# nekStab/neklab

Measured on AMD Instinct MI355X. Metric: linop matvecs/sec + Arnoldi iter time, E=10k N=7, 1/2/4/8 GPU, higher is better.
Workload: dtype f64

## Files before the change

### include/neklab_gpu.h

```cpp
#ifndef NEKLAB_GPU_H
#define NEKLAB_GPU_H

#include <stddef.h>
#include <stdint.h>

#ifdef __cplusplus
extern "C" {
#endif

typedef struct nlg_ctx nlg_ctx;
typedef struct nlg_mesh nlg_mesh;
typedef struct nlg_vec nlg_vec;
typedef struct nlg_basis nlg_basis;
typedef struct nlg_linop nlg_linop;

enum { NLG_VX = 0, NLG_VY = 1, NLG_VZ = 2, NLG_PR = 3, NLG_THETA = 4  };

const char *nlg_last_error(void);
int nlg_version(void);
int nlg_ctx_create(int device, nlg_ctx **out);
int nlg_ctx_destroy(nlg_ctx *ctx);
int nlg_ctx_sync(nlg_ctx *ctx);
int nlg_comm_unique_id(void *out128);
int nlg_ctx_comm_init(nlg_ctx *ctx, int rank, int nranks, const void *unique_id128);
int nlg_ctx_rank(const nlg_ctx *ctx, int *rank, int *nranks);
int nlg_ctx_comm_init_shm(nlg_ctx *ctx, int rank, int nranks, const char *name, int64_t slot_bytes);
int64_t nlg_halo_plan(int rank, int nranks, const int64_t *counts, const int64_t *labels_concat,
                      int64_t *neigh_counts, int64_t *shared_out, int64_t capacity);
int64_t nlg_halo_boundary_labels(int n, int dim, int64_t E, const int64_t *glo, int64_t *labels_out, int64_t capacity);
int64_t nlg_halo_lists(int n, int dim, int64_t E, const int64_t *glo, int rank, int nranks, const int64_t *counts,
                       const int64_t *labels_concat, int64_t *neigh_counts, int32_t *send_idx, int64_t cap_send,
                       int32_t *roff, int32_t *rpos, int32_t *coff, int32_t *cidx, int64_t cap_copies, int64_t *nlab_out);
int nlg_prof_enable(nlg_ctx *ctx, int class_mask);
int nlg_prof_sample(nlg_ctx *ctx, int stride);
int nlg_prof_reset(nlg_ctx *ctx);
int nlg_prof_get(nlg_ctx *ctx, const char *name, int64_t *count, double *total_ms);
int nlg_counters(int64_t *launches, int64_t *collectives);

typedef struct nlg_mesh_desc {
    int dim;
    int n;
    int lxd;
    int64_t nelv;
    const double *xm1;
    const double *ym1;
    const double *zm1;
    const int64_t *glo_num;
    const int64_t *lglel;
    const double *v1mask;
    const double *v2mask;
    const double *v3mask;
    const double *tmask;
    int has_outflow;
} nlg_mesh_desc;

int nlg_mesh_create(nlg_ctx *ctx, const nlg_mesh_desc *desc, nlg_mesh **out);
int nlg_mesh_destroy(nlg_mesh *mesh);
int nlg_mesh_sizes(const nlg_mesh *mesh, int64_t *lvn, int64_t *lpn, int *dim, int *n);
int nlg_mesh_get(const nlg_mesh *mesh, const char *name, double *out, int64_t count);

int nlg_vec_create(nlg_mesh *mesh, int nscal, int lorder, nlg_vec **out);
int nlg_vec_destroy(nlg_vec *v);
int nlg_vec_generation(const nlg_vec *v, int64_t *gen);
int nlg_vec_release(nlg_vec *v);
int nlg_vec_adopt(nlg_vec *v, int64_t gen, int *status);
int nlg_vec_pin(nlg_vec *v, int64_t gen);
int nlg_vec_unpin(nlg_vec *v, int64_t gen);
int nlg_vec_pool_limit(int64_t bytes);
int nlg_vec_pool_trim(int64_t *freed_bytes);
int nlg_vec_clone(const nlg_vec *src, nlg_vec **out);
int nlg_vec_copy(nlg_vec *dst, const nlg_vec *src);
int nlg_vec_zero(nlg_vec *self);
int nlg_vec_rand(nlg_vec *self, int ifnorm, uint64_t seed);
int nlg_vec_rand_noise(nlg_vec *self, uint64_t seed);
int nlg_vec_rand_finish(nlg_vec *self, int ifnorm);
int nlg_vec_scal(nlg_vec *self, double alpha);
int nlg_vec_axpby(double alpha, const nlg_vec *vec, double beta, nlg_vec *self);
int nlg_vec_dot(const nlg_vec *self, const nlg_vec *vec, double *out);
int nlg_vec_norm(const nlg_vec *self, double *out);
int nlg_vec_size(const nlg_vec *self, int64_t *out);
int64_t nlg_vec_size_value(const nlg_vec *self);
int nlg_vec_has_rst_value(const nlg_vec *self);
int64_t nlg_vec_size_checked(const nlg_vec *self, int64_t gen);
int nlg_vec_has_rst_checked(const nlg_vec *self, int64_t gen);
int nlg_vec_outpost(const nlg_vec *self, const char *path, int with_coords, double time, int istep);
int nlg_vec_save_rst(nlg_vec *self, const nlg_vec *vec_rst, int irst);
int nlg_vec_get_rst(const nlg_vec *self, nlg_vec *vec_rst, int irst);
int nlg_vec_has_rst_fields(const nlg_vec *self, int *out);
int nlg_vec_clear_rst_fields(nlg_vec *self);
int nlg_vec_nrst(const nlg_vec *self, int *out);
int nlg_vec_set_field(nlg_vec *self, int field, int irst, const double *host, int64_t count);
int nlg_vec_get_field(const nlg_vec *self, int field, int irst, double *host, int64_t count);
int nlg_set_axpby_rst_consistent(int flag);

int nlg_basis_create(nlg_mesh *mesh, int nscal, int lorder, int nvec, nlg_basis **out);
int nlg_basis_destroy(nlg_basis *b);
int nlg_basis_vec(nlg_basis *b, int i, nlg_vec **out);
int nlg_basis_block_dot(const nlg_basis *b, int k, const nlg_vec *w, double *h);
int nlg_basis_block_axpy(const nlg_basis *b, int k, const double *h, nlg_vec *w);
int nlg_basis_cgs2(const nlg_basis *b, int k, nlg_vec *w, double *h, double *beta);
int nlg_basis_block_cgs2(nlg_basis *b, int k, int s, double *coef);
int nlg_basis_last_block_rank(const nlg_basis *b, int *rank);
int nlg_basis_combine(const nlg_basis *b, int k, const double *c, nlg_vec *out);

typedef struct nlg_exptA_config {
    double tau;
    double re;
    double cfl_limit;
    double vtol;
    double ptol;
    double dt;
    int torder;
// ... 96 lines not shown
```

### neklab_amd/_lib.py

```python
from __future__ import annotations

import ctypes as C
import os

HERE = os.path.dirname(os.path.abspath(__file__))
LIB_PATH = os.path.join(HERE, "libneklab_gpu.so")

c_double_p = C.POINTER(C.c_double)
c_int64_p = C.POINTER(C.c_int64)
c_int_p = C.POINTER(C.c_int)
vp = C.c_void_p


class NlgError(RuntimeError):
    pass


class MeshDesc(C.Structure):
    _fields_ = [
        ("dim", C.c_int), ("n", C.c_int), ("lxd", C.c_int), ("nelv", C.c_int64),
        ("xm1", c_double_p), ("ym1", c_double_p), ("zm1", c_double_p),
        ("glo_num", c_int64_p), ("lglel", c_int64_p),
        ("v1mask", c_double_p), ("v2mask", c_double_p), ("v3mask", c_double_p), ("tmask", c_double_p),
        ("has_outflow", C.c_int),
# ... 7 lines not shown
        ("torder", C.c_int), ("maxit_v", C.c_int), ("maxit_p", C.c_int),
        ("fixed_iters_v", C.c_int), ("fixed_iters_p", C.c_int), ("pprecond", C.c_int), ("pproj", C.c_int),
        ("ifheat", C.c_int), ("conductivity", C.c_double), ("rhocp", C.c_double), ("buoy", C.c_double * 3),
        ("no_history", C.c_int),
        ("filter_weight", C.c_double), ("filter_modes", C.c_int),
    ]


class EigsOpts(C.Structure):
    _fields_ = [
        ("kdim", C.c_int), ("transpose", C.c_int), ("max_restarts", C.c_int), ("write_intermediate", C.c_int),
        ("tol", C.c_double), ("logfile", C.c_char_p), ("seed", C.c_uint64), ("block_size", C.c_int), ("warm_start", C.c_int),
    ]


class OtdOpts(C.Structure):
    _fields_ = [("r", C.c_int), ("startstep", C.c_int), ("orthostep", C.c_int), ("trans", C.c_int), ("solve_baseflow", C.c_int)]


SIGNATURES = {
    "nlg_last_error": (C.c_char_p, []),
    "nlg_version": (C.c_int, []),
    "nlg_ctx_create": (C.c_int, [C.c_int, C.POINTER(vp)]),
    "nlg_ctx_destroy": (C.c_int, [vp]),
    "nlg_ctx_sync": (C.c_int, [vp]),
    "nlg_comm_unique_id": (C.c_int, [vp]),
    "nlg_ctx_comm_init": (C.c_int, [vp, C.c_int, C.c_int, vp]),
    "nlg_ctx_rank": (C.c_int, [vp, c_int_p, c_int_p]),
    "nlg_ctx_comm_init_shm": (C.c_int, [vp, C.c_int, C.c_int, C.c_char_p, C.c_int64]),
    "nlg_halo_plan": (C.c_int64, [C.c_int, C.c_int, c_int64_p, c_int64_p, c_int64_p, c_int64_p, C.c_int64]),
    "nlg_halo_boundary_labels": (C.c_int64, [C.c_int, C.c_int, C.c_int64, c_int64_p, c_int64_p, C.c_int64]),
    "nlg_halo_lists": (C.c_int64, [C.c_int, C.c_int, C.c_int64, c_int64_p, C.c_int, C.c_int, c_int64_p, c_int64_p, c_int64_p,
                                   C.POINTER(C.c_int32), C.c_int64, C.POINTER(C.c_int32), C.POINTER(C.c_int32), C.POINTER(C.c_int32),
                                   C.POINTER(C.c_int32), C.c_int64, c_int64_p]),
    "nlg_prof_enable": (C.c_int, [vp, C.c_int]),
    "nlg_prof_sample": (C.c_int, [vp, C.c_int]),
    "nlg_prof_reset": (C.c_int, [vp]),
    "nlg_prof_get": (C.c_int, [vp, C.c_char_p, c_int64_p, c_double_p]),
    "nlg_counters": (C.c_int, [c_int64_p, c_int64_p]),
    "nlg_basis_last_block_rank": (C.c_int, [vp, C.POINTER(C.c_int)]),
    "nlg_vec_generation": (C.c_int, [vp, c_int64_p]),
    "nlg_vec_release": (C.c_int, [vp]),
    "nlg_vec_adopt": (C.c_int, [vp, C.c_int64, C.POINTER(C.c_int)]),
    "nlg_vec_pin": (C.c_int, [vp, C.c_int64]),
    "nlg_vec_unpin": (C.c_int, [vp, C.c_int64]),
    "nlg_vec_size_checked": (C.c_int64, [vp, C.c_int64]),
    "nlg_vec_has_rst_checked": (C.c_int, [vp, C.c_int64]),
    "nlg_vec_pool_limit": (C.c_int, [C.c_int64]),
    "nlg_vec_pool_trim": (C.c_int, [c_int64_p]),
    "nlg_mesh_create": (C.c_int, [vp, C.POINTER(MeshDesc), C.POINTER(vp)]),
    "nlg_mesh_destroy": (C.c_int, [vp]),
    "nlg_mesh_sizes": (C.c_int, [vp, c_int64_p, c_int64_p, c_int_p, c_int_p]),
    "nlg_mesh_get": (C.c_int, [vp, C.c_char_p, c_double_p, C.c_int64]),
    "nlg_vec_create": (C.c_int, [vp, C.c_int, C.c_int, C.POINTER(vp)]),
    "nlg_vec_destroy": (C.c_int, [vp]),
    "nlg_vec_clone": (C.c_int, [vp, C.POINTER(vp)]),
    "nlg_vec_copy": (C.c_int, [vp, vp]),
    "nlg_vec_zero": (C.c_int, [vp]),
    "nlg_vec_rand": (C.c_int, [vp, C.c_int, C.c_uint64]),
    "nlg_vec_rand_noise": (C.c_int, [vp, C.c_uint64]),
    "nlg_vec_size_value": (C.c_int64, [vp]),
    "nlg_vec_has_rst_value": (C.c_int, [vp]),
    "nlg_basis_block_cgs2": (C.c_int, [vp, C.c_int, C.c_int, c_double_p]),
    "nlg_linop_matvec_block": (C.c_int, [vp, C.c_int, C.POINTER(vp), C.POINTER(vp), C.c_int]),
    "nlg_block_arnoldi_step": (C.c_int, [vp, vp, C.c_int, C.c_int, c_double_p, C.c_int, C.c_int]),
    "nlg_vec_outpost": (C.c_int, [vp, C.c_char_p, C.c_int, C.c_double, C.c_int]),
    "nlg_vec_rand_finish": (C.c_int, [vp, C.c_int]),
    "nlg_vec_scal": (C.c_int, [vp, C.c_double]),
    "nlg_vec_axpby": (C.c_int, [C.c_double, vp, C.c_double, vp]),
    "nlg_vec_dot": (C.c_int, [vp, vp, c_double_p]),
    "nlg_vec_norm": (C.c_int, [vp, c_double_p]),
    "nlg_vec_size": (C.c_int, [vp, c_int64_p]),
    "nlg_vec_save_rst": (C.c_int, [vp, vp, C.c_int]),
    "nlg_vec_get_rst": (C.c_int, [vp, vp, C.c_int]),
    "nlg_vec_has_rst_fields": (C.c_int, [vp, c_int_p]),
    "nlg_vec_clear_rst_fields": (C.c_int, [vp]),
    "nlg_vec_nrst": (C.c_int, [vp, c_int_p]),
    "nlg_vec_set_field": (C.c_int, [vp, C.c_int, C.c_int, c_double_p, C.c_int64]),
    "nlg_vec_get_field": (C.c_int, [vp, C.c_int, C.c_int, c_double_p, C.c_int64]),
    "nlg_set_axpby_rst_consistent": (C.c_int, [C.c_int]),
    "nlg_basis_create": (C.c_int, [vp, C.c_int, C.c_int, C.c_int, C.POINTER(vp)]),
    "nlg_basis_destroy": (C.c_int, [vp]),
    "nlg_basis_vec": (C.c_int, [vp, C.c_int, C.POINTER(vp)]),
    "nlg_basis_block_dot": (C.c_int, [vp, C.c_int, vp, c_double_p]),
    "nlg_basis_block_axpy": (C.c_int, [vp, C.c_int, c_double_p, vp]),
    "nlg_basis_cgs2": (C.c_int, [vp, C.c_int, vp, c_double_p, c_double_p]),
    "nlg_basis_combine": (C.c_int, [vp, C.c_int, c_double_p, vp]),
    "nlg_exptA_config_default": (C.c_int, [C.POINTER(ExptAConfig)]),
    "nlg_linop_create": (C.c_int, [vp, C.POINTER(ExptAConfig), vp, C.POINTER(vp)]),
    "nlg_linop_destroy": (C.c_int, [vp]),
    "nlg_linop_init": (C.c_int, [vp]),
    "nlg_linop_nonlinear_map": (C.c_int, [vp, vp, vp]),
    "nlg_linop_set_baseflow": (C.c_int, [vp, vp]),
    "nlg_linop_set_tolerances": (C.c_int, [vp, C.c_double, C.c_double]),
    "nlg_linop_set_projection": (C.c_int, [vp, C.c_double, C.c_int, c_int64_p, c_int64_p, c_double_p]),
    "nlg_linop_project": (C.c_int, [vp, vp]),
    "nlg_linop_integrate_forced": (C.c_int, [vp, vp, vp, vp, C.c_double, C.c_int, vp]),
    "nlg_linop_matvec": (C.c_int, [vp, vp, vp]),
    "nlg_linop_rmatvec": (C.c_int, [vp, vp, vp]),
    "nlg_linop_set_tau": (C.c_int, [vp, C.c_double]),
    "nlg_linop_set_orbit": (C.c_int, [vp, vp, C.c_double]),
    "nlg_linop_orbit_end": (C.c_int, [vp, vp]),
    "nlg_linop_lane_iters": (C.c_int, [vp, C.c_int, C.c_int, c_int64_p, c_int64_p]),
    "nlg_linop_pcg_z_free": (C.c_int, [vp, c_int_p]),
    "nlg_linop_set_orbit_steps": (C.c_int, [vp, vp, C.c_double, C.c_int]),
    "nlg_upo_residual": (C.c_int, [vp, vp]),
# ... 60 lines not shown
```

### neklab_amd/csrc/internal.h

```cpp
#pragma once
#include <hip/hip_runtime.h>
#include <rccl/rccl.h>

#include <cstdint>
#include <cstdio>
#include <cstring>
#include <map>
#include <string>
#include <vector>

#include "neklab_gpu.h"

namespace nlg {

void set_error(const char *fmt, ...);

#define NLG_HIP(call)                                                                            \
    do {                                                                                         \
        hipError_t e_ = (call);                                                                  \
        if (e_ != hipSuccess) {                                                                  \
            nlg::set_error("%s:%d: %s -> %s", __FILE__, __LINE__, #call, hipGetErrorString(e_)); \
            return 1;                                                                            \
        }                                                                                        \
    } while (0)
// ... 294 lines not shown
int allreduce_max(nlg_ctx *ctx, double *d_buf, int count);
int allgather_f64(nlg_ctx *ctx, const double *d_in, double *d_out, int64_t count);
int shm_allreduce(nlg_ctx *ctx, double *d_buf, int count, bool is_max);
int shm_allgather_i64(nlg_ctx *ctx, const int64_t *d_in, int64_t *d_out, int64_t count);
int shm_exchange(nlg_ctx *ctx, const nlg_halo &h, int nf, hipStream_t st);
void shm_close(nlg_ctx *ctx);

int basis_block_dot_dev(const nlg_basis *b, int k, const nlg_vec *w, double *d_out, double *d_acc);
int basis_block_axpy_dev(const nlg_basis *b, int k, const double *d_h, nlg_vec *w, double sign, const double *d_hh = nullptr,
                         bool main_only = false);
int basis_cgs2_dev(nlg_basis *b, int k, nlg_vec *w);

int pprec_setup(nlg_mesh *m, const nlg_mesh_desc *d);
struct nlg_pcg_upd {
    const double *alpha = nullptr, *wmean = nullptr;
    double *x = nullptr;
    const double *p = nullptr, *w = nullptr, *nw = nullptr;
    double *rr_part = nullptr;
};
int pprec_apply(nlg_mesh *m, hipStream_t st, const double *flag, const double *r, double *z, double *rz_part, bool overlap,
                bool with_coarse, const nlg_pcg_upd *upd = nullptr, int nl = 1, int64_t ld = 0);
int pprec_reserve_lanes(nlg_mesh *m, int nl);
void pprec_free(nlg_mesh *m);

int halo_setup(nlg_mesh *m, const int64_t *glo_num);
int halo_exchange(nlg_mesh *m, double *const *fields, int nf, int layout = 0, int nl = 1, int64_t ld = 0, bool assign = false);
int gs_split(nlg_mesh *m);
int halo_begin(nlg_mesh *m, double *const *fields, int nf, int layout, int nl = 1, int64_t ld = 0);
int halo_finish(nlg_mesh *m, double *const *fields, int nf, int layout, int nl = 1, int64_t ld = 0, bool assign = false);
void halo_free(nlg_mesh *m);

int sem_gs(nlg_mesh *m, double *const *fields, int nf, const double *gate = nullptr, int layout = 0, int nl = 1, int64_t ld = 0, int64_t ldg = 0);
int sem_to_xp(nlg_mesh *m, double *const *src, double *const *dst, int nf, int nl = 1, int64_t ld = 0, double *const *wts = nullptr);
int sem_from_xp(nlg_mesh *m, double *const *src, double *const *dst, int nf, int nl = 1, int64_t ld = 0);
int sem_axhelm(nlg_mesh *m, double *const *u, double *const *w, int nf, double h1, double h2, double *pw_part = nullptr,
               double *const *zf = nullptr, const double *beta_p = nullptr, const double *done_p = nullptr, bool xp = false, int nl = 1, int64_t ld = 0, int64_t uoff = 0,
               const double *pcinv = nullptr, const unsigned char *pcmb = nullptr);
bool sem_axhelm_forms_z(const nlg_mesh *m);
int sem_opdiv_blocks(const nlg_mesh *m);
int sem_axhelm_blocks(nlg_mesh *m, int nf);
int sem_helm_diag(nlg_mesh *m, double *out, double h1, double h2);
struct nlg_pupd {
    const double *z = nullptr, *beta = nullptr, *zmean = nullptr;
    double *p = nullptr;
};
bool sem_opgradt_has_fg(const nlg_mesh *m);
int sem_opgradt(nlg_mesh *m, const double *p, double *const *w, bool face_grouped = false, const double *gate = nullptr, const nlg_pupd *upd = nullptr,
                int nl = 1, int64_t ld = 0, int64_t ldv = 0);
int sem_opdiv(nlg_mesh *m, double *const *u, double *out, double scale, double *const *wts = nullptr, bool face_grouped = false,
              const double *pdot = nullptr, double *pw_part = nullptr, const double *gate = nullptr, int nl = 1, int64_t ld = 0, int64_t ldv = 0);
int sem_opbinv(nlg_mesh *m, double *const *w, int nl = 1, int64_t ld = 0);
bool sem_opgradt_fuses_pupdate(const nlg_mesh *m);
bool sem_small_mesh(const nlg_mesh *m);
int sem_cdabdtp(nlg_mesh *m, const double *p, double *out, double *pw_part = nullptr, const double *gate = nullptr, const nlg_pupd *upd = nullptr,
                int nl = 1, int64_t ld = 0);
int sem_ediag(nlg_mesh *m, double *out);
int sem_tensor(nlg_mesh *m, const double *in, double *out, int nin, int nout, const double *Mx, const double *My,
               const double *Mz, const double *wt);
int sem_conv_setup(nlg_mesh *m, double *const *U, double **Ur, double **GU);
int sem_conv_apply(nlg_mesh *m, double *const *Ur, double *const *GU, double *const *u, double *const *out, int adjoint, int nl = 1, int64_t ld = 0);
int sem_conv_apply_generic(nlg_mesh *m, double *const *Ur, double *const *GU, double *const *u, double *const *out, int adjoint);
int sem_conv_scalar_setup(nlg_mesh *m, const double *Theta, double **GT);
int sem_conv_scalar_apply(nlg_mesh *m, double *const *Ur, double *const *GT, double *const *u, const double *theta, double *out, int adjoint = 0,
                          int nl = 1, int64_t ld = 0);
int sem_scalar_grad_apply(nlg_mesh *m, double *const *GT, const double *theta, double *const *out, double sgn, int nl = 1, int64_t ld = 0);
int sem_cfl(nlg_mesh *m, double *const *U, double dt, double *cfl_host);
int sem_ortho(nlg_mesh *m, double *p, int nl = 1, int64_t ld = 0);
bool sem_filter_available(const nlg_mesh *m);
int sem_filter_matrix(const nlg_mesh *m, int ncut, double weight, std::vector<double> &F);
int sem_filter(nlg_mesh *m, const double *F, double *const *fields, int nf, int nl = 1, int64_t ld = 0, double *const *upd_x = nullptr,
               double *const *upd_wt = nullptr, double upd_s = 0.0, const int *slot = nullptr);
double *sem_scratch1(nlg_mesh *m, int i);
double *sem_scratchd(nlg_mesh *m, int i);
double *sem_scratch2(nlg_mesh *m, int i);

}
```

### neklab_amd/csrc/sem.hip

```cpp
#include <algorithm>
#include <cmath>
#include <numeric>

#include <type_traits>

#include "internal.h"

using namespace nlg;

namespace {

void legendre(int N, double x, double &pN, double &pNm1) {
    double p0 = 1.0, p1 = x;
    if (N == 0) {
        pN = 1.0;
        pNm1 = 0.0;
        return;
    }
    for (int k = 2; k <= N; ++k) {
        const double p2 = ((2 * k - 1) * x * p1 - (k - 1) * p0) / k;
        p0 = p1;
        p1 = p2;
    }
    pN = p1;
// ... 3195 lines not shown
    NLG_CHECK(!beta_p || (zf && done_p), "sem_axhelm: the fused direction update needs zf and the done flag");
    CF3 cz = {{zf ? zf[0] : nullptr, (zf && nf > 1) ? zf[1] : nullptr, (zf && nf > 2) ? zf[2] : nullptr}};
    if (m->dim == 3) {
#define AX3(N_)                                                                                                       \
    {                                                                                                                 \
        const int64_t tot = m->E * nf;                                                                                \
        const int *tab = xp ? (const int *)m->d_slot_xp : nullptr;                                                    \
        if constexpr (N_ <= 8) {                                                                                      \
            const dim3 grid((unsigned)((tot + kAxhelm3rWaves - 1) / kAxhelm3rWaves), nl), block(64 * kAxhelm3rWaves); \
            if (xp)                                                                                                   \
                NLG_LAUNCH((k_axhelm3r<N_, true>), grid, block, 0, s, m->E, nf, m->d_D, m->d_G[0], m->d_G[1], m->d_G[2], m->d_G[3], m->d_G[4], m->d_G[5], m->d_bm1, cu, cw, h1, h2, pw_part, cz, beta_p, done_p, tab, ld, uoff, pcinv, pcmb); \
            else                                                                                                      \
                NLG_LAUNCH((k_axhelm3r<N_, false>), grid, block, 0, s, m->E, nf, m->d_D, m->d_G[0], m->d_G[1], m->d_G[2], m->d_G[3], m->d_G[4], m->d_G[5], m->d_bm1, cu, cw, h1, h2, pw_part, cz, beta_p, done_p, tab, ld, uoff, pcinv, pcmb); \
        } else {                                                                                                      \
            constexpr int PPB_ = axhelm3c_ppb(N_);                                                                    \
            const dim3 grid((unsigned)((tot + PPB_ - 1) / PPB_), nl), block(((PPB_ * N_ * N_ + 63) / 64) * 64);       \
            if (xp)                                                                                                   \
                NLG_LAUNCH((k_axhelm3c<N_, true, PPB_>), grid, block, 0, s, m->E, nf, m->d_D, m->d_G[0], m->d_G[1], m->d_G[2], m->d_G[3], m->d_G[4], m->d_G[5], m->d_bm1, cu, cw, h1, h2, pw_part, cz, beta_p, done_p, tab, ld, uoff, pcinv, pcmb); \
            else                                                                                                      \
                NLG_LAUNCH((k_axhelm3c<N_, false, PPB_>), grid, block, 0, s, m->E, nf, m->d_D, m->d_G[0], m->d_G[1], m->d_G[2], m->d_G[3], m->d_G[4], m->d_G[5], m->d_bm1, cu, cw, h1, h2, pw_part, cz, beta_p, done_p, tab, ld, uoff, pcinv, pcmb); \
        }                                                                                                             \
    }
        NLG_FOR_N(AX3)
#undef AX3
    } else {
#define AX2(N_)                                                                                                       \
    {                                                                                                                 \
        constexpr int EPB = (NT / (N_ * N_)) > 0 ? (NT / (N_ * N_)) : 1;                                              \
        const int grid = (int)((m->E + EPB - 1) / EPB);                                                               \
        if (nf == 1)                                                                                                  \
            NLG_LAUNCH((k_axhelm2<N_, 1>), dim3(grid), dim3(EPB * N_ * N_), 0, s, m->E, m->d_D, m->d_G[0],     \
                               m->d_G[1], m->d_G[2], m->d_bm1, cu, cw, h1, h2, pw_part, cz, beta_p, done_p, uoff);                                 \
        else if (nf == 2)                                                                                             \
            NLG_LAUNCH((k_axhelm2<N_, 2>), dim3(grid), dim3(EPB * N_ * N_), 0, s, m->E, m->d_D, m->d_G[0],     \
                               m->d_G[1], m->d_G[2], m->d_bm1, cu, cw, h1, h2, pw_part, cz, beta_p, done_p, uoff);                                 \
        else                                                                                                          \
            NLG_LAUNCH((k_axhelm2<N_, 3>), dim3(grid), dim3(EPB * N_ * N_), 0, s, m->E, m->d_D, m->d_G[0],     \
                               m->d_G[1], m->d_G[2], m->d_bm1, cu, cw, h1, h2, pw_part, cz, beta_p, done_p, uoff);                                 \
    }
        NLG_FOR_N(AX2)
#undef AX2
    }
    NLG_HIP(hipGetLastError());
    return 0;
}

int sem_helm_diag(nlg_mesh *m, double *out, double h1, double h2) {
    NLG_LAUNCH(k_helm_diag, dim3(grid_for(m->lvn)), dim3(NT), 0, m->ctx->stream, m->dim, m->n, m->E, m->d_D,
                       m->d_G[0], m->d_G[1], m->d_G[2], m->d_G[3], m->d_G[4], m->d_G[5], m->d_bm1, out, h1, h2);
    NLG_HIP(hipGetLastError());
    return 0;
}

template <int N>
static void fill_pmats(const nlg_mesh *m, PMats<N> &M) {
    const int n2 = N - 2;
    const nlg_ops1d &o = m->ops;
    for (int k = 0; k < n2; ++k)
        for (int j = 0; j < N; ++j) {
            M.Im[k * N + j] = o.I12[(size_t)k * N + j];
            M.Dm[k * N + j] = o.D12[(size_t)k * N + j];
            M.It[j * n2 + k] = o.I12[(size_t)k * N + j];
            M.Dt[j * n2 + k] = o.D12[(size_t)k * N + j];
        }
}

bool sem_small_mesh(const nlg_mesh *m) {
    static const int64_t lim = getenv("NLG_SMALL_E") ? atoll(getenv("NLG_SMALL_E")) : 4096;
    return m->E < lim;
}

static CF9 rst2w_ptrs(const nlg_mesh *m) {
    CF9 g;
    for (int q = 0; q < 9; ++q) g.p[q] = m->d_rst2w[q];
    return g;
}

template <typename T>
static T *at_lane(T *p, int v, int64_t ld) {
    return p ? p + v * ld : nullptr;
}
static F3 at_lane3(double *const *a, int nf, int v, int64_t ld) {
    F3 r = {{nullptr, nullptr, nullptr}};
    for (int c = 0; c < nf; ++c) r.p[c] = at_lane(a[c], v, ld);
    return r;
}

bool sem_opgradt_fuses_pupdate(const nlg_mesh *m) { return m->dim == 3 && m->n >= 8 && m->n <= 10; }

int sem_opgradt(nlg_mesh *m, const double *p, double *const *w, bool face_grouped, const double *gate, const nlg_pupd *upd, int nl, int64_t ld,
                int64_t ldv) {
    NLG_CHECK(!upd || sem_opgradt_fuses_pupdate(m), "sem_opgradt: the fused direction update exists for 3-D, lx1 >= 8 only");
    PUpd pu;
    for (int v = 0; v < 4; ++v) {
        const bool on = upd && v < nl && upd->z;
        pu.z[v] = on ? at_lane(upd->z, v, ld) : nullptr;
        pu.beta[v] = on ? at_lane(upd->beta, v, ld) : nullptr;
        pu.zmean[v] = on ? at_lane(upd->zmean, v, ld) : nullptr;
        pu.p[v] = on ? at_lane(upd->p, v, ld) : nullptr;
    }
    ProfScope ps(m->ctx, (m->dim == 2 || face_grouped) ? P_OPGRADT : P_VECOPS);
    CF9 g = rst2w_ptrs(m);
    hipStream_t s = m->ctx->stream;
    if (m->dim == 3) {
        CP4 pl, gl;
        F3L wl;
        for (int v = 0; v < 4; ++v) {
            pl.p[v] = v < nl ? p + v * ld : nullptr;
            gl.p[v] = v < nl ? at_lane(gate, v, ld) : nullptr;
            for (int c = 0; c < 3; ++c) wl.p[v][c] = v < nl ? at_lane(w[c], v, ldv) : nullptr;
        }
        if (m->n == 8 && nl == 1 && sem_small_mesh(m)) {
            const F3 w3 = {{w[0], w[1], w[2]}};
            if (upd) {
                if (face_grouped)
                    NLG_LAUNCH((k_opgradt3w<8, true, true>), dim3((unsigned)m->E), dim3(192), 0, s, m->E, (const double *)m->d_I12t, (const double *)m->d_D12t, (const int *)m->d_slot_fg, g, p, w3, gate, pu);
                else
                    NLG_LAUNCH((k_opgradt3w<8, false, true>), dim3((unsigned)m->E), dim3(192), 0, s, m->E, (const double *)m->d_I12t, (const double *)m->d_D12t, (const int *)m->d_slot_fg, g, p, w3, gate, pu);
            } else {
                if (face_grouped)
                    NLG_LAUNCH((k_opgradt3w<8, true, false>), dim3((unsigned)m->E), dim3(192), 0, s, m->E, (const double *)m->d_I12t, (const double *)m->d_D12t, (const int *)m->d_slot_fg, g, p, w3, gate, NoPUpd{});
                else
                    NLG_LAUNCH((k_opgradt3w<8, false, false>), dim3((unsigned)m->E), dim3(192), 0, s, m->E, (const double *)m->d_I12t, (const double *)m->d_D12t, (const int *)m->d_slot_fg, g, p, w3, gate, NoPUpd{});
            }
            NLG_HIP(hipGetLastError());
            return 0;
        }
#define GT3_(N_, ML_)                                                                                                        \
    if constexpr (N_ < 8) {                                                                                            \
        PMats<N_> M;                                                                                                   \
        fill_pmats<N_>(m, M);                                                                                          \
        if (face_grouped)                                                                                              \
            NLG_LAUNCH((k_opgradt3<N_, true, ML_>), dim3((unsigned)m->E), dim3(NT), 0, s, m->E, M, g, pl, wl, gl, nl);       \
        else                                                                                                           \
            NLG_LAUNCH((k_opgradt3<N_, false, ML_>), dim3((unsigned)m->E), dim3(NT), 0, s, m->E, M, g, pl, wl, gl, nl);      \
    } else if (face_grouped) {                                                                                         \
        if (upd)                                                                                                       \
            NLG_LAUNCH((k_opgradt3n<(N_ <= 10 ? N_ : 9), true, ML_, true>), dim3((unsigned)m->E), dim3(PBlockN<N_>::NTB), 0, s, m->E, (const double *)m->d_I12t, (const double *)m->d_D12t, (const int *)m->d_slot_fg, g, pl, wl, gl, nl, pu);    \
        else                                                                                                           \
            NLG_LAUNCH((k_opgradt3n<N_, true, ML_, false>), dim3((unsigned)m->E), dim3(PBlockN<N_>::NTB), 0, s, m->E, (const double *)m->d_I12t, (const double *)m->d_D12t, (const int *)m->d_slot_fg, g, pl, wl, gl, nl, NoPUpd{});    \
    } else {                                                                                                           \
        if (upd)                                                                                                       \
            NLG_LAUNCH((k_opgradt3n<(N_ <= 10 ? N_ : 9), false, ML_, true>), dim3((unsigned)m->E), dim3(PBlockN<N_>::NTB), 0, s, m->E, (const double *)m->d_I12t, (const double *)m->d_D12t, (const int *)m->d_slot_fg, g, pl, wl, gl, nl, pu);   \
        else                                                                                                           \
            NLG_LAUNCH((k_opgradt3n<N_, false, ML_, false>), dim3((unsigned)m->E), dim3(PBlockN<N_>::NTB), 0, s, m->E, (const double *)m->d_I12t, (const double *)m->d_D12t, (const int *)m->d_slot_fg, g, pl, wl, gl, nl, NoPUpd{});   \
    }
#define GT3(N_)           \
    if (nl == 1) {        \
        GT3_(N_, false)   \
    } else {              \
        GT3_(N_, true)    \
    }
        NLG_FOR_N(GT3)
#undef GT3
#undef GT3_
    } else {
        for (int v = 0; v < nl; ++v) {
            F3 cw = {{w[0] + v * ldv, w[1] + v * ldv, nullptr}};
            const double *pv = p + v * ld;
#define GT2(N_)                                                                                              \
    {                                                                                                        \
        constexpr int EPB = NT / (N_ * N_) > 0 ? NT / (N_ * N_) : 1;                                         \
        NLG_LAUNCH((k_opgradt2<N_>), dim3((unsigned)((m->E + EPB - 1) / EPB)), dim3(NT), 0, s, m->E, \
                           m->d_I12t, m->d_D12t, g, pv, cw);                                                 \
    }
            NLG_FOR_N(GT2)
#undef GT2
        }
    }
    NLG_HIP(hipGetLastError());
    return 0;
}

int sem_opdiv_blocks(const nlg_mesh *m) {
    if (m->dim == 3) return (int)m->E;
    const int epb = NT / (m->n * m->n) > 0 ? NT / (m->n * m->n) : 1;
    return (int)((m->E + epb - 1) / epb);
}

int sem_opdiv(nlg_mesh *m, double *const *u, double *out, double scale, double *const *wts, bool face_grouped, const double *pdot, double *pw_part,
              const double *gate, int nl, int64_t ld, int64_t ldv) {
    ProfScope ps(m->ctx, (m->dim == 2 || face_grouped) ? P_OPDIV : P_VECOPS);
    CF3 wt = {{wts ? wts[0] : nullptr, wts ? wts[1] : nullptr, (wts && m->dim == 3) ? wts[2] : nullptr}};
    static const bool use_mb = !(getenv("NLG_OPDIV_MASKB") && atoi(getenv("NLG_OPDIV_MASKB")) == 0);
    const unsigned char *mb = nullptr;
    CF3 wtn = wt;
    if (use_mb && m->dim == 3 && face_grouped && wts == m->d_mbinv_fg && m->d_maskb_fg && m->d_binv_fg) {
        mb = m->d_maskb_fg;
        wtn.p[0] = m->d_binv_fg;
        wtn.p[1] = wtn.p[2] = nullptr;
    }
    CF9 g = rst2w_ptrs(m);
    hipStream_t s = m->ctx->stream;
    if (m->dim == 3) {
        CF3L ul;
        P4 ol, pl;
        CP4 dl, gl;
        for (int v = 0; v < 4; ++v) {
            for (int c = 0; c < 3; ++c) ul.p[v][c] = v < nl ? at_lane(u[c], v, ldv) : nullptr;
            ol.p[v] = v < nl ? out + v * ld : nullptr;
            pl.p[v] = v < nl ? at_lane(pw_part, v, ld) : nullptr;
            dl.p[v] = v < nl ? at_lane(pdot, v, ld) : nullptr;
            gl.p[v] = v < nl ? at_lane(gate, v, ld) : nullptr;
        }
        if (m->n == 8 && nl == 1 && sem_small_mesh(m)) {
            const CF3 u3 = {{u[0], u[1], u[2]}};
            if (face_grouped)
                NLG_LAUNCH((k_opdiv3w<8, true>), dim3((unsigned)m->E), dim3(192), 0, s, m->E, (const double *)m->d_I12, (const double *)m->d_D12, (const int *)m->d_slot_fg, g, u3, wt, out, scale, pdot, pw_part, gate);
            else
                NLG_LAUNCH((k_opdiv3w<8, false>), dim3((unsigned)m->E), dim3(192), 0, s, m->E, (const double *)m->d_I12, (const double *)m->d_D12, (const int *)m->d_slot_fg, g, u3, wt, out, scale, pdot, pw_part, gate);
            NLG_HIP(hipGetLastError());
            return 0;
        }
#define DV3_(N_, ML_)                                                                                                        \
    if constexpr (N_ < 8) {                                                                                            \
        PMats<N_> M;                                                                                                   \
        fill_pmats<N_>(m, M);                                                                                          \
        if (face_grouped)                                                                                              \
            NLG_LAUNCH((k_opdiv3<N_, true, ML_>), dim3((unsigned)m->E), dim3(NT), 0, s, m->E, M, g, ul, wt, ol, scale, dl, pl, gl, nl);  \
        else                                                                                                           \
            NLG_LAUNCH((k_opdiv3<N_, false, ML_>), dim3((unsigned)m->E), dim3(NT), 0, s, m->E, M, g, ul, wt, ol, scale, dl, pl, gl, nl); \
    } else if (face_grouped)                                                                                           \
        NLG_LAUNCH((k_opdiv3n<N_, true, ML_>), dim3((unsigned)m->E), dim3(PBlockN<N_>::NTB), 0, s, m->E, (const double *)m->d_I12, (const double *)m->d_D12, (const int *)m->d_slot_fg, g, ul, wtn, ol, scale, dl, pl, gl, nl, mb);  \
    else                                                                                                               \
        NLG_LAUNCH((k_opdiv3n<N_, false, ML_>), dim3((unsigned)m->E), dim3(PBlockN<N_>::NTB), 0, s, m->E, (const double *)m->d_I12, (const double *)m->d_D12, (const int *)m->d_slot_fg, g, ul, wtn, ol, scale, dl, pl, gl, nl, mb);
#define DV3(N_)           \
    if (nl == 1) {        \
        DV3_(N_, false)   \
    } else {              \
        DV3_(N_, true)    \
    }
        NLG_FOR_N(DV3)
#undef DV3
#undef DV3_
    } else {
        for (int v = 0; v < nl; ++v) {
            CF3 cu = {{u[0] + v * ldv, u[1] + v * ldv, nullptr}};
            double *ov = out + v * ld, *pv = at_lane(pw_part, v, ld);
            const double *dv = at_lane(pdot, v, ld), *gv = at_lane(gate, v, ld);
#define DV2(N_)                                                                                            \
    {                                                                                                      \
        constexpr int EPB = NT / (N_ * N_) > 0 ? NT / (N_ * N_) : 1;                                       \
        NLG_LAUNCH((k_opdiv2<N_>), dim3((unsigned)((m->E + EPB - 1) / EPB)), dim3(NT), 0, s, m->E, \
                           m->d_I12, m->d_D12, g, cu, wt, ov, scale, dv, pv, gv);                          \
    }
            NLG_FOR_N(DV2)
#undef DV2
        }
    }
    NLG_HIP(hipGetLastError());
    return 0;
}

int sem_opbinv(nlg_mesh *m, double *const *w, int nl, int64_t ld) {
    NLG_TRY(sem_gs(m, w, m->dim, nullptr, LAYOUT_NAT, nl, ld, 0));
    ProfScope ps(m->ctx, P_COLMUL);
    F3 cw = {{w[0], w[1], m->dim == 3 ? w[2] : nullptr}};
    CF3 wt = {{m->d_mbinv[0], m->d_mbinv[1], m->d_mbinv[2]}};
    if (m->dim == 3)
        NLG_LAUNCH(k_colmul<3>, dim3(grid_for(m->lvn), nl), dim3(NT), 0, m->ctx->stream, cw, wt, m->lvn, ld);
    else
        NLG_LAUNCH(k_colmul<2>, dim3(grid_for(m->lvn), nl), dim3(NT), 0, m->ctx->stream, cw, wt, m->lvn, ld);
    NLG_HIP(hipGetLastError());
    return 0;
}

bool sem_opgradt_has_fg(const nlg_mesh *m) { return m->dim == 3 && m->gs.d_indices_fg && m->d_slot_fg && (!m->halo.active || m->halo.d_send_idx_fg); }
// ... 882 lines not shown
    if (!m) return 0;
    hipDeviceSynchronize();
    nlg_vec_pool_trim(nullptr);
    double *ptrs[] = {m->d_D, m->d_Dt, m->d_I12, m->d_I12t, m->d_D12, m->d_D12t, m->d_Jd, m->d_Jdt, m->d_DJd, m->d_DJdt,
                      m->d_rdr, m->d_w1, m->d_w2, m->d_wd, m->d_jac, m->d_bm1, m->d_binvm1, m->d_vmult, m->d_tmask,
                      m->d_bm2, m->d_bm2inv};
    for (double *p : ptrs)
        if (p) hipFree(p);
    for (int c = 0; c < 3; ++c) {
        if (m->d_x[c]) hipFree(m->d_x[c]);
        if (m->d_mask[c]) hipFree(m->d_mask[c]);
        if (m->d_mbinv[c]) hipFree(m->d_mbinv[c]);
    }
    for (int q = 0; q < 9; ++q) {
        if (m->d_rst[q]) hipFree(m->d_rst[q]);
        if (m->d_rst2w[q]) hipFree(m->d_rst2w[q]);
        if (m->d_rstdw[q]) hipFree(m->d_rstdw[q]);
    }
    for (int q = 0; q < 6; ++q)
        if (m->d_G[q]) hipFree(m->d_G[q]);
    if (m->d_lglel) hipFree(m->d_lglel);
    halo_free(m);
    pprec_free(m);
    if (m->d_binv_fg) hipFree(m->d_binv_fg);
    if (m->d_maskb_fg) hipFree(m->d_maskb_fg);
    if (m->d_slot_fg) hipFree(m->d_slot_fg);
    if (m->gs.d_offsets_fg) hipFree(m->gs.d_offsets_fg);
    if (m->gs.d_indices_fg) hipFree(m->gs.d_indices_fg);
    if (m->gs.d_offsets_xp) hipFree(m->gs.d_offsets_xp);
    if (m->gs.d_indices_xp) hipFree(m->gs.d_indices_xp);
    if (m->d_slot_xp) hipFree(m->d_slot_xp);
    if (m->d_vmult_xp) hipFree(m->d_vmult_xp);
    if (m->d_wlanes) hipFree(m->d_wlanes);
    for (int c = 0; c < 3; ++c)
        if (m->d_mbinv_fg[c]) hipFree(m->d_mbinv_fg[c]);
    if (m->gs.d_offsets) hipFree(m->gs.d_offsets);
    if (m->gs.d_indices) hipFree(m->gs.d_indices);
    for (double *p : m->scratch1) hipFree(p);
    for (double *p : m->scratch2) hipFree(p);
    for (double *p : m->scratchd) hipFree(p);
    delete m;
    return 0;
}

int nlg_mesh_sizes(const nlg_mesh *m, int64_t *lvn, int64_t *lpn, int *dim, int *n) {
    NLG_CHECK(m, "nlg_mesh_sizes: NULL mesh");
    if (lvn) *lvn = m->lvn;
    if (lpn) *lpn = m->lpn;
    if (dim) *dim = m->dim;
    if (n) *n = m->n;
    return 0;
}

int nlg_mesh_get(const nlg_mesh *m, const char *name, double *out, int64_t count) {
    NLG_CHECK(m && name && out, "nlg_mesh_get: NULL argument");
    if (strcmp(name, "ediag") == 0) {
        NLG_CHECK(count == m->lpn, "nlg_mesh_get: count mismatch for ediag");
        nlg_mesh *mm = const_cast<nlg_mesh *>(m);
        double *ed = sem_scratch2(mm, 5);
        NLG_TRY(sem_ediag(mm, ed));
        NLG_HIP(hipMemcpyAsync(out, ed, sizeof(double) * (size_t)m->lpn, hipMemcpyDeviceToHost, m->ctx->stream));
        NLG_HIP(hipStreamSynchronize(m->ctx->stream));
        return 0;
    }
    if (strncmp(name, "hdiag:", 6) == 0) {
        double h1 = 0, h2 = 0;
        NLG_CHECK(sscanf(name + 6, "%lf:%lf", &h1, &h2) == 2, "nlg_mesh_get: bad hdiag spec '%s'", name);
        NLG_CHECK(count == m->lvn, "nlg_mesh_get: count mismatch for hdiag");
        nlg_mesh *mm = const_cast<nlg_mesh *>(m);
        double *dg = sem_scratch1(mm, 3);
        NLG_TRY(sem_helm_diag(mm, dg, h1, h2));
        double *f[1] = {dg};
        NLG_TRY(sem_gs(mm, f, 1));
        NLG_HIP(hipMemcpyAsync(out, dg, sizeof(double) * (size_t)m->lvn, hipMemcpyDeviceToHost, m->ctx->stream));
        NLG_HIP(hipStreamSynchronize(m->ctx->stream));
        return 0;
    }
    auto it = m->named.find(name);
    NLG_CHECK(it != m->named.end(), "nlg_mesh_get: unknown array '%s'", name);
    const int64_t len = m->named_len.at(name);
    NLG_CHECK(count == len, "nlg_mesh_get: count %lld != length %lld of '%s'", (long long)count, (long long)len, name);
    NLG_HIP(hipMemcpyAsync(out, it->second, sizeof(double) * (size_t)len, hipMemcpyDeviceToHost, m->ctx->stream));
    NLG_HIP(hipStreamSynchronize(m->ctx->stream));
    return 0;
}

int nlg_vec_rand(nlg_vec *self, int ifnorm, uint64_t seed) {
    NLG_TRY(nlg_vec_rand_noise(self, seed));
    return nlg_vec_rand_finish(self, ifnorm);
}

int nlg_vec_rand_noise(nlg_vec *self, uint64_t seed) {
    NLG_CHECK(self, "nlg_vec_rand: NULL vector");
    nlg_mesh *m = self->mesh;
    hipStream_t s = m->ctx->stream;
    CF3 X = {{m->d_x[0], m->d_x[1], m->d_x[2]}};
    for (int f = 0; f < self->ncomp; ++f) {
        double *fld = f < m->dim ? self->vel(f) : self->theta(f - m->dim);
        NLG_LAUNCH(k_rand_add, dim3(grid_for(m->lvn)), dim3(NT), 0, s, m->dim, m->n, m->E, m->d_lglel, X, fld, f, seed);
    }
    NLG_HIP(hipGetLastError());
    return 0;
}

int nlg_vec_rand_finish(nlg_vec *self, int ifnorm) {
    NLG_CHECK(self, "nlg_vec_rand: NULL vector");
// ... 218 lines not shown
```

### neklab_amd/host.py

```python
from __future__ import annotations

import ctypes as C
import os

import numpy as np

from . import _lib
from ._lib import NlgError, check, dptr, vp

VX, VY, VZ, PR, THETA = 0, 1, 2, 3, 4


class Context:

    def __init__(self, device: int = 0):
        self.lib = _lib.load()
        h = vp()
        check(self.lib.nlg_ctx_create(int(device), C.byref(h)))
        self.h = h
        self.rank, self.nranks = 0, 1

    def comm_init(self, rank: int, nranks: int, unique_id: bytes):
        buf = C.create_string_buffer(unique_id, 128)
        check(self.lib.nlg_ctx_comm_init(self.h, rank, nranks, C.cast(buf, vp)))
# ... 10 lines not shown
        check(lib.nlg_comm_unique_id(C.cast(buf, vp)))
        return buf.raw

    def sync(self):
        check(self.lib.nlg_ctx_sync(self.h))

    def close(self):
        if self.h:
            self.lib.nlg_ctx_destroy(self.h)
            self.h = None


class Mesh:

    def __init__(self, ctx: Context, mesh, lxd: int = 0):
        self.ctx, self.lib = ctx, ctx.lib
        self.host = mesh
        d = _lib.MeshDesc()
        d.dim, d.n, d.lxd, d.nelv = mesh.dim, mesh.n, int(lxd), mesh.E
        keep = []

        def f64(a):
            a = np.ascontiguousarray(a, dtype=np.float64)
            keep.append(a)
            return dptr(a)

        d.xm1, d.ym1 = f64(mesh.x), f64(mesh.y)
        d.zm1 = f64(mesh.z) if mesh.dim == 3 else None
        g = np.ascontiguousarray(mesh.glo_num, dtype=np.int64)
        keep.append(g)
        d.glo_num = g.ctypes.data_as(_lib.c_int64_p)
        if mesh.elem_gid is not None:
            eg = np.ascontiguousarray(mesh.elem_gid, dtype=np.int64)
            keep.append(eg)
            d.lglel = eg.ctypes.data_as(_lib.c_int64_p)
        d.v1mask, d.v2mask = f64(mesh.mask[0]), f64(mesh.mask[1])
        d.v3mask = f64(mesh.mask[2]) if mesh.dim == 3 else None
        d.tmask = f64(mesh.tmask)
        d.has_outflow = int(mesh.has_outflow)
        h = vp()
        check(self.lib.nlg_mesh_create(ctx.h, C.byref(d), C.byref(h)))
        self.h = h
        lvn, lpn = C.c_int64(), C.c_int64()
        check(self.lib.nlg_mesh_sizes(h, C.byref(lvn), C.byref(lpn), None, None))
        self.lvn, self.lpn = lvn.value, lpn.value
        self.dim, self.n = mesh.dim, mesh.n
        self.E = mesh.E

    def get(self, name: str, on_mesh: int = 1) -> np.ndarray:
        npts = {1: self.lvn, 2: self.lpn}.get(on_mesh, on_mesh)
        out = np.empty(npts)
        check(self.lib.nlg_mesh_get(self.h, name.encode(), dptr(out), npts))
        return out

    def close(self):
        if self.h:
            self.lib.nlg_mesh_destroy(self.h)
            self.h = None

    def __del__(self):
        try:
            self.close()
        except Exception:
            pass


class nek_dvector:

    def __init__(self, mesh: Mesh, nscal: int = 0, lorder: int = 3, _handle=None, _owns=True):
        self.mesh, self.lib = mesh, mesh.lib
        self.nscal, self.lorder = nscal, lorder
        self._owns = _owns
        if _handle is None:
            h = vp()
            check(self.lib.nlg_vec_create(mesh.h, nscal, lorder, C.byref(h)))
            self.h = h
        else:
            self.h = _handle

    def zero(self):
        check(self.lib.nlg_vec_zero(self.h))

    def rand(self, ifnorm: bool = False, seed: int = 0):
        check(self.lib.nlg_vec_rand(self.h, int(bool(ifnorm)), int(seed)))

    def scal(self, alpha: float):
        check(self.lib.nlg_vec_scal(self.h, float(alpha)))

    def axpby(self, alpha: float, vec: "nek_dvector", beta: float):
        if not isinstance(vec, nek_dvector):
            raise TypeError("type_error: vec must be nek_dvector (reference: real_vectors.f90:202-204)")
        check(self.lib.nlg_vec_axpby(float(alpha), vec.h, float(beta), self.h))

    def dot(self, vec: "nek_dvector") -> float:
        if not isinstance(vec, nek_dvector):
            raise TypeError("type_error: vec must be nek_dvector (reference: real_vectors.f90:229-231)")
        out = C.c_double()
        check(self.lib.nlg_vec_dot(self.h, vec.h, C.byref(out)))
        return out.value

    def get_size(self) -> int:
        out = C.c_int64()
        check(self.lib.nlg_vec_size(self.h, C.byref(out)))
        return out.value

    def norm(self) -> float:
# ... 1016 lines not shown
```

Baseline: 23.54.

## Add MFMA-based opgradt and opdiv kernels for 3D N=8 pressure operators

```diff
diff --git a/include/neklab_gpu.h b/include/neklab_gpu.h
--- a/include/neklab_gpu.h
+++ b/include/neklab_gpu.h
@@ -58,6 +58,7 @@
 int nlg_mesh_destroy(nlg_mesh *mesh);
 int nlg_mesh_sizes(const nlg_mesh *mesh, int64_t *lvn, int64_t *lpn, int *dim, int *n);
 int nlg_mesh_get(const nlg_mesh *mesh, const char *name, double *out, int64_t count);
+int nlg_mesh_pop_mfma(const nlg_mesh *mesh, int *out);
 
 int nlg_vec_create(nlg_mesh *mesh, int nscal, int lorder, nlg_vec **out);
 int nlg_vec_destroy(nlg_vec *v);
diff --git a/neklab_amd/_lib.py b/neklab_amd/_lib.py
--- a/neklab_amd/_lib.py
+++ b/neklab_amd/_lib.py
@@ -83,6 +83,7 @@
     "nlg_mesh_destroy": (C.c_int, [vp]),
     "nlg_mesh_sizes": (C.c_int, [vp, c_int64_p, c_int64_p, c_int_p, c_int_p]),
     "nlg_mesh_get": (C.c_int, [vp, C.c_char_p, c_double_p, C.c_int64]),
+    "nlg_mesh_pop_mfma": (C.c_int, [vp, c_int_p]),
     "nlg_vec_create": (C.c_int, [vp, C.c_int, C.c_int, C.POINTER(vp)]),
     "nlg_vec_destroy": (C.c_int, [vp]),
     "nlg_vec_clone": (C.c_int, [vp, C.POINTER(vp)]),
diff --git a/neklab_amd/csrc/internal.h b/neklab_amd/csrc/internal.h
--- a/neklab_amd/csrc/internal.h
+++ b/neklab_amd/csrc/internal.h
@@ -370,6 +370,7 @@
 int sem_opbinv(nlg_mesh *m, double *const *w, int nl = 1, int64_t ld = 0);
 bool sem_opgradt_fuses_pupdate(const nlg_mesh *m);
 bool sem_small_mesh(const nlg_mesh *m);
+bool sem_pop_mfma(const nlg_mesh *m);
 int sem_cdabdtp(nlg_mesh *m, const double *p, double *out, double *pw_part = nullptr, const double *gate = nullptr, const nlg_pupd *upd = nullptr,
                 int nl = 1, int64_t ld = 0);
 int sem_ediag(nlg_mesh *m, double *out);
diff --git a/neklab_amd/csrc/sem.hip b/neklab_amd/csrc/sem.hip
--- a/neklab_amd/csrc/sem.hip
+++ b/neklab_amd/csrc/sem.hip
@@ -3271,6 +3271,302 @@
     return 0;
 }
 
+namespace {
+__device__ __forceinline__ v4f64 mfma4(double a, double b, v4f64 c) { return __builtin_amdgcn_mfma_f64_16x16x4f64(a, b, c, 0, 0, 0); }
+__device__ __forceinline__ double ld_off(const double *base, unsigned off) { return *(const double *)((const char *)base + off); }
+
+template <bool FG, bool PU>
+__global__ __launch_bounds__(64, 4) void k_opgradt3m8(int64_t E, const double *__restrict__ mIt, const double *__restrict__ mDt, const int *__restrict__ fgtab, CF9 g,
+                                                   const double *__restrict__ p, F3 w, const double *__restrict__ gate, std::conditional_t<PU, PUpd, NoPUpd> pu) {
+    constexpr int N = 8, N2 = 6, NS2 = 36, NP2 = 216, NP1 = 512, RW = 54, RY = 54;
+    __shared__ double sS[18 * RW];
+    if (gate && gate[0] != 0.0) return;
+    const int lane = threadIdx.x, l15 = lane & 15, lg = lane >> 4, r8 = l15 & 7;
+    const bool top = l15 < 8, lo = lg < 2;
+    const int64_t e = blockIdx.x;
+    const v4f64 zero = {0.0, 0.0, 0.0, 0.0};
+    const int kA = lg, kB = 4 + (lg & 1);
+    const double zA0 = top ? mIt[r8 * N2 + kA] : 0.0;
+    const double zA1 = lo ? (top ? mIt[r8 * N2 + kB] : 0.0) : (top ? 0.0 : mDt[r8 * N2 + kB]);
+    const double zA2 = top ? 0.0 : mDt[r8 * N2 + kA];
+    double yA[5];
+    int yoff[5];
+#pragma unroll
+    for (int s = 0; s < 5; ++s) {
+        const bool pad = s == 4 && (lg & 1);
+        const int kr = s < 4 ? (2 * s + (lg >> 1)) + 8 * (lg & 1) : 16 + (lg >> 1);
+        const int arr = kr / N2, j2 = kr % N2;
+        const double v = top ? (arr == 0 ? mIt[r8 * N2 + j2] : 0.0) : (arr == 1 ? mDt[r8 * N2 + j2] : (arr == 2 ? mIt[r8 * N2 + j2] : 0.0));
+        yA[s] = pad ? 0.0 : v;
+        yoff[s] = kr * RW + l15;
+    }
+    double xM[3];
+    int xoff[3];
+#pragma unroll
+    for (int s = 0; s < 3; ++s) {
+        const int kr = 4 * s + lg, b = kr / N2, i2 = kr % N2;
+        xM[s] = b == 0 ? mDt[r8 * N2 + i2] : mIt[r8 * N2 + i2];
+        xoff[s] = (b * N + 2 * (l15 & 3)) * RY + (l15 >> 2) * N2 + i2;
+    }
+    int ia[3], ib[3], zw[3];
+    bool cv[3];
+    double pA[3], pB[3];
+    const double *pe = p + e * NP2;
+#pragma unroll
+    for (int t = 0; t < 3; ++t) {
+        const int col = 16 * t + l15, cc = col < NS2 ? col : NS2 - 1;
+        cv[t] = col < NS2;
+        ia[t] = cc + NS2 * kA;
+        ib[t] = cc + NS2 * kB;
+        zw[t] = (cc / N2) * RW + cc % N2;
+        pA[t] = pe[ia[t]];
+        pB[t] = pe[ib[t]];
+    }
+    if constexpr (PU) if (pu.z[0]) {
+        const double beta = pu.beta[0][0], zmean = pu.zmean[0][0];
+        const double *ze = pu.z[0] + e * NP2;
+        double *po = pu.p[0] + e * NP2;
+        double zvA[3], zvB[3];
+#pragma unroll
+        for (int t = 0; t < 3; ++t) {
+            zvA[t] = ze[ia[t]];
+            zvB[t] = ze[ib[t]];
+        }
+#pragma unroll
+        for (int t = 0; t < 3; ++t) {
+            pA[t] = (zvA[t] - zmean) + beta * pA[t];
+            pB[t] = (zvB[t] - zmean) + beta * pB[t];
+            if (cv[t]) po[ia[t]] = pA[t];
+            if (cv[t] && lo) po[ib[t]] = pB[t];
+        }
+    }
+#pragma unroll
+    for (int t = 0; t < 3; ++t)
+        if (!cv[t]) pA[t] = pB[t] = 0.0;
+    double gq[3][5];
+    auto load_g = [&](int i) {
+        const double *g0 = g.p[i] + e * NP2, *g1 = g.p[3 + i] + e * NP2, *g2 = g.p[6 + i] + e * NP2;
+        const double *gx = lo ? g0 : g2;
+#pragma unroll
+        for (int t = 0; t < 3; ++t) {
+            gq[t][0] = g0[ia[t]];
+            gq[t][1] = g2[ia[t]];
+            gq[t][2] = g1[ia[t]];
+            gq[t][3] = gx[ib[t]];
+            gq[t][4] = g1[ib[t]];
+        }
+    };
+    load_g(0);
+#pragma unroll 1
+    for (int i = 0; i < 3; ++i) {
+        if (i > 0) lds_barrier();
+#pragma unroll
+        for (int t = 0; t < 3; ++t) {
+            v4f64 d = mfma4(zA0, gq[t][0] * pA[t], zero);
+            d = mfma4(zA1, gq[t][3] * pB[t], d);
+            d = mfma4(zA2, gq[t][1] * pA[t], d);
+            v4f64 d1 = mfma4(zA0, gq[t][2] * pA[t], zero);
+            d1 = mfma4(zA1, lo ? gq[t][4] * pB[t] : 0.0, d1);
+            if (cv[t]) {
+                double *r = sS + zw[t] + N2 * lg;
+                r[0] = d[0];
+                r[4 * N2] = d[1];
+                r[N2 * RW] = d1[0];
+                r[N2 * RW + 4 * N2] = d1[1];
+                r[2 * N2 * RW] = d[2];
+                r[2 * N2 * RW + 4 * N2] = d[3];
+            }
+        }
+        if (i < 2) load_g(i + 1);
+        lds_barrier();
+#pragma unroll
+        for (int t = 0; t < 3; ++t) {
+            double yb[5];
+#pragma unroll
+            for (int s = 0; s < 5; ++s) yb[s] = sS[yoff[s] + 16 * t];
+            v4f64 d = mfma4(yA[0], yb[0], zero);
+#pragma unroll
+            for (int s = 1; s < 5; ++s) d = mfma4(yA[s], yb[s], d);
+            double *r = sS + lg * RY + 16 * t + l15;
+            r[0] = d[0];
+            r[4 * RY] = d[1];
+            r[8 * RY] = d[2];
+            r[12 * RY] = d[3];
+        }
+        lds_barrier();
+        double *wp = w.p[i] + e * NP1;
+        int sl[2][4];
+#pragma unroll
+        for (int t = 0; t < 2; ++t)
+#pragma unroll
+            for (int r = 0; r < 4; ++r) sl[t][r] = FG ? fgtab[lane + 64 * (4 * t + r)] : lane + 64 * (4 * t + r);
+#pragma unroll
+        for (int t = 0; t < 2; ++t) {
+            v4f64 d = zero;
+#pragma unroll
+            for (int s = 0; s < 3; ++s) d = mfma4(sS[xoff[s] + 4 * t * N2], top ? xM[s] : 0.0, d);
+#pragma unroll
+            for (int s = 0; s < 3; ++s) d = mfma4(sS[xoff[s] + RY + 4 * t * N2], top ? 0.0 : xM[s], d);
+#pragma unroll
+            for (int r = 0; r < 4; ++r) wp[sl[t][r]] = d[r];
+        }
+    }
+}
+
+__global__ __launch_bounds__(64, 4) void k_opdiv3m8(int64_t E, const double *__restrict__ mIm, const double *__restrict__ mDm, const int *__restrict__ fgtab, CF9 g, CF3 u,
+                                                 const double *__restrict__ binv, const unsigned char *__restrict__ mb, double *__restrict__ out, double scale,
+                                                 const double *__restrict__ pdot, double *__restrict__ part, const double *__restrict__ gate) {
+    constexpr int N = 8, N2 = 6, NS2 = 36, NP2 = 216, NP1 = 512, RW = 54, RY = 54;
+    __shared__ double sS[18 * RW];
+    if (gate && gate[0] != 0.0) return;
+    const int lane = threadIdx.x, l15 = lane & 15, lg = lane >> 4, r8 = l15 & 7;
+    const bool top = l15 < 8, lo = lg < 2;
+    const int64_t e = blockIdx.x;
+    const v4f64 zero = {0.0, 0.0, 0.0, 0.0};
+    const int r6 = r8 < N2 ? r8 : N2 - 1;
+    const double live = r8 < N2 ? 1.0 : 0.0;
+    const double aA = live * (top ? mDm[r6 * N + lg] : mIm[r6 * N + lg]);
+    const double aB = live * (top ? mDm[r6 * N + lg + 4] : mIm[r6 * N + lg + 4]);
+    const int jx = l15 >> 3, kx = l15 & 7;
+    const int cw = lane + (lane >> 3), cr = lg + 9 * jx + 72 * kx;
+    int ia[3], ib[3], zr[3];
+    bool cv[3];
+#pragma unroll
+    for (int t = 0; t < 3; ++t) {
+        const int col = 16 * t + l15, cc = col < NS2 ? col : NS2 - 1;
+        cv[t] = col < NS2;
+        ia[t] = cc + NS2 * lg;
+        ib[t] = cc + NS2 * (4 + (lg & 1));
+        zr[t] = (cc / N2) * RW + cc % N2 + N2 * lg;
+    }
+    double acc[3][2];
+#pragma unroll
+    for (int t = 0; t < 3; ++t) acc[t][0] = acc[t][1] = 0.0;
+    unsigned so[N];
+#pragma unroll
+    for (int u8 = 0; u8 < N; ++u8) so[u8] = 8u * (unsigned)fgtab[lane + 64 * u8];
+    double ww[N];
+    unsigned mk = 0u;
+    {
+        const double *wq = binv + e * NP1;
+        const unsigned char *mp = mb + e * NP1;
+#pragma unroll
+        for (int u8 = 0; u8 < N; ++u8) {
+            ww[u8] = ld_off(wq, so[u8]);
+            mk |= (unsigned)(mp[so[u8] >> 3] & 7u) << (3 * u8);
+        }
+    }
+#pragma unroll 1
+    for (int i = 0; i < 3; ++i) {
+        if (i > 0) lds_barrier();
+        const double *up = u.p[i] + e * NP1;
+        double uu[N];
+#pragma unroll
+        for (int u8 = 0; u8 < N; ++u8) uu[u8] = ld_off(up, so[u8]);
+#pragma unroll
+        for (int u8 = 0; u8 < N; ++u8) uu[u8] *= ((mk >> (3 * u8 + i)) & 1u) ? ww[u8] : 0.0;
+#pragma unroll
+        for (int u8 = 0; u8 < N; ++u8) sS[cw + 72 * u8] = uu[u8];
+        lds_barrier();
+        double xb[4][2];
+#pragma unroll
+        for (int t = 0; t < 4; ++t) {
+            xb[t][0] = sS[cr + 18 * t];
+            xb[t][1] = sS[cr + 18 * t + 4];
+        }
+#pragma unroll
+        for (int t = 0; t < 4; ++t) {
+            v4f64 d = mfma4(aA, xb[t][0], zero);
+            d = mfma4(aB, xb[t][1], d);
+            double *r = sS + (2 * t + jx) * RY + kx * N2 + lg;
+            r[0] = d[0];
+            r[N * RY] = d[2];
+            if (lo) {
+                r[4] = d[1];
+                r[N * RY + 4] = d[3];
+            }
+        }
+        double gq[3][3][2];
+#pragma unroll
+        for (int j = 0; j < 3; ++j) {
+            const double *gp = g.p[j * 3 + i] + e * NP2;
+#pragma unroll
+            for (int t = 0; t < 3; ++t) {
+                gq[j][t][0] = gp[ia[t]];
+                gq[j][t][1] = gp[ib[t]];
+            }
+        }
+        lds_barrier();
+#pragma unroll
+        for (int t = 0; t < 3; ++t) {
+            double yb[4];
+#pragma unroll
+            for (int s = 0; s < 4; ++s) yb[s] = sS[(4 * s + lg) * RY + 16 * t + l15];
+            v4f64 d0 = mfma4(aA, yb[0], zero);
+            d0 = mfma4(aB, yb[1], d0);
+            v4f64 d1 = mfma4(aA, yb[2], zero);
+            d1 = mfma4(aB, yb[3], d1);
+            double *r = sS + lg * RW + 16 * t + l15;
+            r[0] = d0[2];
+            r[N2 * RW] = d1[0];
+            r[2 * N2 * RW] = d1[2];
+            if (lo) {
+                r[4 * RW] = d0[3];
+                r[(N2 + 4) * RW] = d1[1];
+                r[(2 * N2 + 4) * RW] = d1[3];
+            }
+        }
+        lds_barrier();
+#pragma unroll
+        for (int j = 0; j < 3; ++j) {
+#pragma unroll
+            for (int t = 0; t < 3; ++t) {
+                const double *r = sS + j * N2 * RW + zr[t];
+                v4f64 d = mfma4(aA, r[0], zero);
+                d = mfma4(aB, r[4 * N2], d);
+                acc[t][0] += gq[j][t][0] * (j < 2 ? d[2] : d[0]);
+                acc[t][1] += gq[j][t][1] * (j < 2 ? d[3] : d[1]);
+            }
+            __builtin_amdgcn_sched_barrier(0);
+        }
+    }
+    double spw = 0.0, sw = 0.0;
+    {
+        double pd[3][2];
+#pragma unroll
+        for (int t = 0; t < 3; ++t) {
+            pd[t][0] = part ? pdot[e * NP2 + ia[t]] : 0.0;
+            pd[t][1] = part ? pdot[e * NP2 + ib[t]] : 0.0;
+        }
+#pragma unroll
+        for (int t = 0; t < 3; ++t) {
+            const double v0 = scale * acc[t][0], v1 = scale * acc[t][1];
+            if (cv[t]) {
+                out[e * NP2 + ia[t]] = v0;
+                spw += pd[t][0] * v0;
+                sw += v0;
+                if (lo) {
+                    out[e * NP2 + ib[t]] = v1;
+                    spw += pd[t][1] * v1;
+                    sw += v1;
+                }
+            }
+        }
+    }
+    if (part) {
+#pragma unroll
+        for (int o = 32; o > 0; o >>= 1) {
+            spw += __shfl_down(spw, o, 64);
+            sw += __shfl_down(sw, o, 64);
+        }
+        if (lane == 0) {
+            part[e] = spw;
+            part[E + e] = sw;
+        }
+    }
+}
+}
+
 template <int N>
 static void fill_pmats(const nlg_mesh *m, PMats<N> &M) {
     const int n2 = N - 2;
@@ -3287,6 +3583,11 @@
 bool sem_small_mesh(const nlg_mesh *m) {
     static const int64_t lim = getenv("NLG_SMALL_E") ? atoll(getenv("NLG_SMALL_E")) : 4096;
     return m->E < lim;
+}
+
+bool sem_pop_mfma(const nlg_mesh *m) {
+    static const bool on = !(getenv("NLG_POP_MFMA") && atoi(getenv("NLG_POP_MFMA")) == 0);
+    return on && m->dim == 3 && m->n == 8 && !sem_small_mesh(m);
 }
 
 static CF9 rst2w_ptrs(const nlg_mesh *m) {
@@ -3345,7 +3646,23 @@
             NLG_HIP(hipGetLastError());
             return 0;
         }
-#define GT3_(N_, ML_)                                                                                                        \
+        if (nl == 1 && sem_pop_mfma(m)) {
+            const F3 w3 = {{w[0], w[1], w[2]}};
+            if (upd) {
+                if (face_grouped)
+                    NLG_LAUNCH((k_opgradt3m8<true, true>), dim3((unsigned)m->E), dim3(64), 0, s, m->E, (const double *)m->d_I12t, (const double *)m->d_D12t, (const int *)m->d_slot_fg, g, p, w3, gate, pu);
+                else
+                    NLG_LAUNCH((k_opgradt3m8<false, true>), dim3((unsigned)m->E), dim3(64), 0, s, m->E, (const double *)m->d_I12t, (const double *)m->d_D12t, (const int *)m->d_slot_fg, g, p, w3, gate, pu);
+            } else {
+                if (face_grouped)
+                    NLG_LAUNCH((k_opgradt3m8<true, false>), dim3((unsigned)m->E), dim3(64), 0, s, m->E, (const double *)m->d_I12t, (const double *)m->d_D12t, (const int *)m->d_slot_fg, g, p, w3, gate, NoPUpd{});
+                else
+                    NLG_LAUNCH((k_opgradt3m8<false, false>), dim3((unsigned)m->E), dim3(64), 0, s, m->E, (const double *)m->d_I12t, (const double *)m->d_D12t, (const int *)m->d_slot_fg, g, p, w3, gate, NoPUpd{});
+            }
+            NLG_HIP(hipGetLastError());
+            return 0;
+        }
+#define GT3_(N_, ML_)                                                                                                       \
     if constexpr (N_ < 8) {                                                                                            \
         PMats<N_> M;                                                                                                   \
         fill_pmats<N_>(m, M);                                                                                          \
@@ -3431,7 +3748,13 @@
             NLG_HIP(hipGetLastError());
             return 0;
         }
-#define DV3_(N_, ML_)                                                                                                        \
+        if (nl == 1 && sem_pop_mfma(m) && mb) {
+            const CF3 u3 = {{u[0], u[1], u[2]}};
+            NLG_LAUNCH(k_opdiv3m8, dim3((unsigned)m->E), dim3(64), 0, s, m->E, (const double *)m->d_I12, (const double *)m->d_D12, (const int *)m->d_slot_fg, g, u3, wtn.p[0], mb, out, scale, pdot, pw_part, gate);
+            NLG_HIP(hipGetLastError());
+            return 0;
+        }
+#define DV3_(N_, ML_)                                                                                                       \
     if constexpr (N_ < 8) {                                                                                            \
         PMats<N_> M;                                                                                                   \
         fill_pmats<N_>(m, M);                                                                                          \
@@ -4420,6 +4743,12 @@
     return 0;
 }
 
+int nlg_mesh_pop_mfma(const nlg_mesh *m, int *out) {
+    NLG_CHECK(m && out, "nlg_mesh_pop_mfma: bad argument");
+    *out = sem_pop_mfma(m) ? 1 : 0;
+    return 0;
+}
+
 int nlg_mesh_get(const nlg_mesh *m, const char *name, double *out, int64_t count) {
     NLG_CHECK(m && name && out, "nlg_mesh_get: NULL argument");
     if (strcmp(name, "ediag") == 0) {
diff --git a/neklab_amd/host.py b/neklab_amd/host.py
--- a/neklab_amd/host.py
+++ b/neklab_amd/host.py
@@ -86,6 +86,11 @@
         out = np.empty(npts)
         check(self.lib.nlg_mesh_get(self.h, name.encode(), dptr(out), npts))
         return out
+
+    def pop_mfma(self) -> int:
+        out = C.c_int()
+        check(self.lib.nlg_mesh_pop_mfma(self.h, C.byref(out)))
+        return out.value
 
     def close(self):
         if self.h:
```

New measurement: 24.01, median of 6. 1.02x the previous value.
